# OllieBoyne/sslap

Measured on AMD Instinct MI355X. Metric: Medges/s (bid-phase CSR nnz/s) + solve ms, N=200k d=0.1% sparse LAP, higher is better.
Workload: dtype f64

## Files before the change

sslap_amd/auction_solve.py:

```python
import ctypes as C
import os

import numpy as np

from . import _lib

_ENV_DEVICE = "MISSLAP_DEVICE"
_ENV_TAIL = "MISSLAP_TAIL_THRESHOLD"


def _options(problem, eps_start, max_iter, device=None, tail_threshold=None, profile=None, force_f64=False,
             input_on_device=False, shard=None, rounds_per_sync=None, tiled_min_k=None, tiled_shape=None, shard_min_k=None,
             engine=None, cand=None, nnz_limit=None, cand_build_max_k=None, cand_refresh=None,
             input_stream=None):
    if problem not in ("min", "max"):
        problem = "max" if problem != "min" else "min"
    o = _lib.Options()
    o.struct_size = C.sizeof(_lib.Options)
    o.device = int(os.environ.get(_ENV_DEVICE, 0)) if device is None else int(device)
    o.maximize = 1 if problem == "max" else 0
    o.eps_start = float(np.float32(eps_start))
    o.max_iter = int(max_iter)
    o.input_on_device = 1 if input_on_device else 0
    o.input_stream = None if input_stream is None else C.c_void_p(int(input_stream))
# ... 10 lines not shown
    o.shard_min_K = 0 if shard_min_k is None else int(shard_min_k)
    c = 1 if cand is None else int(cand)
    o.cand_mode = 1 if c == 0 else (2 if c == 2 else 0)
    o.partial_in_list_order = 0
    o.cand_build_max_K = 0 if cand_build_max_k is None else int(cand_build_max_k)
    o.cand_refresh_min = 0 if cand_refresh is None else int(cand_refresh) + 1
    o.nnz_limit = 0 if nnz_limit is None else int(nnz_limit)
    return o


class AuctionSolver:

    def __init__(self, loc, val, num_rows=0, num_cols=0, problem="min", max_iter=1000000, eps_start=0,
                 **gpu_opts):
        lib = _lib.load()
        loc, val = self._check_buffers(loc, val)
        self._h = C.c_void_p()
        self._opts = _options(problem, eps_start, max_iter, **gpu_opts)
        self._problem = problem
        loc_c = np.ascontiguousarray(loc)
        val_c = np.ascontiguousarray(val)
        _lib.check(lib.misslap_create(C.byref(self._h), loc_c.shape[0], loc_c.ctypes.data, val_c.ctypes.data,
                                      C.byref(self._opts)))
        if problem == "min":
            np.multiply(val, -1, out=val)
        self._post_create()

    @classmethod
    def _from_handle(cls, handle, opts, problem):
        self = cls.__new__(cls)
        self._h, self._opts, self._problem = handle, opts, problem
        self._post_create()
        return self

    @classmethod
    def from_dense(cls, mat, problem="min", max_iter=1000000, eps_start=0, **gpu_opts):
        lib = _lib.load()
        h = C.c_void_p()
        opts = _options(problem, eps_start, max_iter, **gpu_opts)
        matc = np.ascontiguousarray(mat)
        nnz = C.c_int64(-1)
        rc = lib.misslap_create_dense(C.byref(h), matc.shape[0], matc.shape[1], matc.ctypes.data, C.byref(opts),
                                      C.byref(nnz))
        return rc, h, opts, int(nnz.value)

    @classmethod
    def from_device_pointers(cls, loc_ptr, val_ptr, nnz, problem="min", max_iter=1000000, eps_start=0,
                             **gpu_opts):
        lib = _lib.load()
        h = C.c_void_p()
        opts = _options(problem, eps_start, max_iter, input_on_device=True, **gpu_opts)
        _lib.check(lib.misslap_create(C.byref(h), int(nnz), C.c_void_p(int(loc_ptr)), C.c_void_p(int(val_ptr)),
                                      C.byref(opts)))
        return cls._from_handle(h, opts, problem)

    @staticmethod
    def _check_buffers(loc, val):
        if not isinstance(loc, np.ndarray) or not isinstance(val, np.ndarray):
            raise TypeError("loc and val must be numpy arrays")
        if loc.ndim != 2:
            raise ValueError(f"Buffer has wrong number of dimensions (expected 2, got {loc.ndim})")
        if loc.dtype != np.int32:
            raise ValueError(f"Buffer dtype mismatch, expected 'DTYPE_int_t' but got '{loc.dtype.name}'")
        if val.ndim != 1:
            raise ValueError(f"Buffer has wrong number of dimensions (expected 1, got {val.ndim})")
        if val.dtype != np.float64:
            raise ValueError(f"Buffer dtype mismatch, expected 'DTYPE_t' but got '{_cname(val.dtype)}'")
        if loc.shape[1] != 2 or loc.shape[0] != val.shape[0]:
            raise ValueError("loc must have shape (nnz, 2) and val shape (nnz,)")
        return loc, val

    def _post_create(self):
        lib = _lib.load()
        n, m, z = C.c_int64(), C.c_int64(), C.c_int64()
        _lib.check(lib.misslap_dims(self._h, C.byref(n), C.byref(m), C.byref(z)))
        self.num_rows, self.num_cols, self.nnz = n.value, m.value, z.value
        st = self.status()
        self.tail_threshold, self.rounds_per_sync = int(st.tail_threshold), int(st.rounds_per_sync)
        self.shard_min_K = int(st.shard_min_K)
        self.meta = {"start_eps": round(float(st.eps), 3)}
        self.gpu = {}

    def __del__(self):
        h = getattr(self, "_h", None)
        if h:
            try:
                _lib.load().misslap_destroy(h)
            except Exception:
                pass
            self._h = None

    def solve(self):
        lib = _lib.load()
        sol = np.empty(self.num_rows, dtype=np.int32)
        meta = _lib.new_meta()
        _lib.check(lib.misslap_solve(self._h, sol.ctypes.data, C.byref(meta)))
        self._fill_meta(meta)
        return sol

    @staticmethod
    def solve_batch(solvers, group_size=0):
        lib = _lib.load()
        n = len(solvers)
        sols = [np.empty(s.num_rows, dtype=np.int32) for s in solvers]
        handles = (C.c_void_p * n)(*[s._h for s in solvers])
        outs = (C.c_void_p * n)(*[a.ctypes.data for a in sols])
        metas = (_lib.Meta * n)()
        for m in metas:
            m.struct_size = C.sizeof(_lib.Meta)
        info = _lib.BatchInfo()
        meta_ptrs = (C.POINTER(_lib.Meta) * n)(*[C.pointer(m) for m in metas])
        _lib.check(lib.misslap_solve_batch(handles, n, outs, meta_ptrs, int(group_size), C.byref(info)))
        for s, m in zip(solvers, metas):
            s._fill_meta(m)
        return sols, dict(groups=int(info.groups), calls_recorded=int(info.calls_recorded),
                          launches_issued=int(info.launches_issued), wall_ms=float(info.wall_ms),
                          host_ms=dict(fibers=round(float(info.host_ms_fibers), 3), flush=round(float(info.host_ms_flush), 3),
                                       wait=round(float(info.host_ms_wait), 3)))

    def solve_sharded(self, comm=None):
        lib = _lib.load()
        sol = np.empty(self.num_rows, dtype=np.int32)
        meta = _lib.new_meta()
        _lib.check(lib.misslap_solve_sharded(self._h, comm._c if comm is not None else None, sol.ctypes.data,
                                             C.byref(meta)))
        self._fill_meta(meta)
        return sol

    def _fill_meta(self, m):
        self.meta["start_eps"] = round(float(m.start_eps), 3)
        self.meta["eCE"] = int(m.eCE)
        self.meta["its"] = int(m.its)
        self.meta["nreductions"] = int(m.nreductions)
        self.meta["soln_found"] = int(m.soln_found)
        self.meta["n_assigned"] = int(m.n_assigned)
        self.meta["obj"] = round(float(m.obj_f32), 3)
        self.meta["final_eps"] = round(float(m.final_eps), 3)
        self.meta["timer"] = {"setup": f"{m.setup_ms:.2f}ms", "solve": f"{m.solve_ms:.2f}ms"}
        g = dict(obj_f64=float(m.obj_f64), edges_scanned=int(m.edges_scanned), bids_made=int(m.bids_made),
                 grid_rounds=int(m.grid_rounds), tail_rounds=int(m.tail_rounds), bytes_per_edge=int(m.bytes_per_edge),
                 setup_ms=float(m.setup_ms), solve_ms=float(m.solve_ms), final_eps_f32=float(m.final_eps),
                 start_eps_f32=float(m.start_eps), tail_edges=int(m.tail_edges), shard_edges=int(m.shard_edges),
                 tiled_active=int(m.tiled_active), tiled_min_K=int(m.tiled_min_K),
                 cand_hits=int(m.cand_hits), cand_edges=int(m.cand_edges), lines_active=int(m.lines_active),
                 sharded_rounds=int(m.sharded_rounds), tiled_format=int(m.tiled_format),
                 phases_with_lines=int(m.phases_with_lines), eps_phases=int(m.eps_phases),
                 filter_undecided=int(m.filter_undecided),
                 complete_assignment=tuple(bool(m.complete_assignment >> k & 1) for k in range(3)),
                 valid_assignment=bool(m.valid_assignment))
        d = [float(x) for x in m.tail_stats]
        g["tail_modes"] = {name: dict(rounds=int(d[k]), ms=round(d[3 + k] * 1e-5, 3),
                                      us_per_round=round(d[3 + k] * 1e-2 / d[k], 3) if d[k] else None)
                           for k, name in enumerate(("solo", "team", "block"))}
        g["tail_cand"] = dict(bids=int(d[6]), hits=int(d[7]), builds=int(d[8]))
        g["tail_cand_edges"] = int(d[9])
        g["tail_raw"] = d[:6]
        if m.profiled:
            g.update(bid_launches=int(m.bid_launches), bid_ms=float(m.bid_ms), bid_edges=int(m.bid_edges),
                     fullscan_launches=int(m.fullscan_launches), fullscan_ms=float(m.fullscan_ms),
                     fullscan_edges=int(m.fullscan_edges), tail_launches=int(m.tail_launches),
                     tail_ms=float(m.tail_ms), tiled_launches=int(m.tiled_launches), tiled_ms=float(m.tiled_ms),
                     tiled_edges=int(m.tiled_edges), bid_edges_read=int(m.bid_edges_read),
                     fullscan_edges_read=int(m.fullscan_edges_read))
        self.gpu = g
        self.meta["gpu"] = g

    @property
    def prices(self):
        p = np.empty(self.num_cols, dtype=np.float64)
        _lib.check(_lib.load().misslap_get_prices(self._h, p.ctypes.data, 0))
        return p

    def update_values(self, val):
        if not isinstance(val, np.ndarray):
            raise TypeError("val must be a numpy array")
        if val.dtype != np.float64:
            raise ValueError(f"Buffer dtype mismatch, expected 'double' but got '{_cname(val.dtype)}'")
        delta = C.c_double(0.0)
        if val.ndim == 2:
            shape = getattr(self, "_dense_shape", None)
            if shape is None:
                raise ValueError("an (N, M) matrix updates a solver made by from_matrix only; pass the nnz values instead")
            if val.shape != shape:
                raise ValueError(f"matrix of shape {val.shape}, the solver was made from one of shape {shape}")
            v = np.ascontiguousarray(val)
            if np.isposinf(v).any():
                raise ValueError("the matrix holds +inf")
            _lib.check(_lib.load().misslap_update_dense(self._h, v.ctypes.data, 0, None, C.byref(delta)))
            return float(delta.value)
        if val.ndim != 1:
            raise ValueError(f"Buffer has wrong number of dimensions (expected 1, got {val.ndim})")
        if val.shape[0] != self.nnz:
            raise ValueError(f"{val.shape[0]} values given, the solver holds {self.nnz} entries")
        v = np.ascontiguousarray(val)
        if not np.isfinite(v).all():
            raise ValueError("val holds a NaN or an infinity")
        _lib.check(_lib.load().misslap_update_values(self._h, v.ctypes.data, self.nnz, 0, None, C.byref(delta)))
        return float(delta.value)

    def update_values_device(self, ptr, input_stream=None, dense=False):
        delta = C.c_double(0.0)
        stream = None if input_stream is None else C.c_void_p(int(input_stream))
        lib = _lib.load()
        if dense:
            _lib.check(lib.misslap_update_dense(self._h, C.c_void_p(int(ptr)), 1, stream, C.byref(delta)))
        else:
            _lib.check(lib.misslap_update_values(self._h, C.c_void_p(int(ptr)), self.nnz, 1, stream, C.byref(delta)))
        return float(delta.value)

    def resolve(self, prices=None, eps_start=0):
        e = float(eps_start)
        if e != e:
            raise ValueError("eps_start is NaN")
        ptr, on_device = None, 0
        if prices is not None:
            if isinstance(prices, np.ndarray):
                if prices.dtype != np.float64:
                    raise ValueError(f"Buffer dtype mismatch, expected 'double' but got '{_cname(prices.dtype)}'")
                p = np.ascontiguousarray(prices)
                bad_nan, bad_sign = not np.isfinite(p).all(), bool(np.signbit(p).any())
                ptr = p.ctypes.data
            elif hasattr(prices, "data_ptr") and getattr(prices, "is_cuda", False):
                import torch
                if prices.dtype != torch.float64:
                    raise ValueError(f"prices must be float64, got {prices.dtype}")
                p = prices.contiguous()
                bad_nan, bad_sign = not bool(torch.isfinite(p).all()), bool(torch.signbit(p).any())
                ptr, on_device = p.data_ptr(), 1
            else:
                raise TypeError("prices must be a numpy array or a tensor on the device")
            if p.ndim != 1 or p.shape[0] != self.num_cols:
                raise ValueError(f"prices must have shape ({self.num_cols},), got {tuple(p.shape)}")
            if bad_nan:
                raise ValueError("prices hold a NaN or an infinity")
            if bad_sign:
                raise ValueError("prices must be >= 0 (with the sign bit clear: -0.0 is rejected)")
        lib = _lib.load()
        sol = np.empty(self.num_rows, dtype=np.int32)
        meta = _lib.new_meta()
        _lib.check(lib.misslap_resolve(self._h, None if ptr is None else C.c_void_p(ptr), on_device, float(np.float32(e)),
                                       sol.ctypes.data, C.byref(meta)))
        self._fill_meta(meta)
        return sol

    def status(self):
        st = _lib.Status()
        _lib.check(_lib.load().misslap_get_status(self._h, C.byref(st)))
        return st

    def state(self):
        st = self.status()
        p = np.empty(self.num_cols, dtype=np.float64)
        U = np.empty(self.num_rows, dtype=np.int32)
        p2o = np.empty(self.num_rows, dtype=np.int32)
        o2p = np.empty(self.num_cols, dtype=np.int32)
        _lib.check(_lib.load().misslap_get_state(self._h, p.ctypes.data, U.ctypes.data, p2o.ctypes.data,
                                                 o2p.ctypes.data))
        return dict(K=int(st.K), U=U[:st.K].copy(), p=p, p2o=p2o, o2p=o2p, eps=float(st.eps), its=int(st.its),
                    nreductions=int(st.nreductions))

    def round_bid(self):
        _lib.check(_lib.load().misslap_round_bid(self._h))

    def round_tiebreak(self):
        _lib.check(_lib.load().misslap_round_tiebreak(self._h))

    def round_apply(self):
        _lib.check(_lib.load().misslap_round_apply(self._h))

    def run_tail(self):
        _lib.check(_lib.load().misslap_run_tail(self._h))

    def phase_end(self):
        fin = C.c_int32(0)
        _lib.check(_lib.load().misslap_phase_end(self._h, C.byref(fin)))
        return bool(fin.value)

    def check_ece(self, eps):
        ok = C.c_int32(0)
        _lib.check(_lib.load().misslap_check_ece(self._h, float(np.float32(eps)), C.byref(ok)))
        return bool(ok.value)

    def finish(self):
        sol = np.empty(self.num_rows, dtype=np.int32)
        meta = _lib.new_meta()
        _lib.check(_lib.load().misslap_finish(self._h, sol.ctypes.data, C.byref(meta)))
        self._fill_meta(meta)
        return sol

    def exchange_buffers(self):
        k, p, n = C.c_void_p(), C.c_void_p(), C.c_int64()
        _lib.check(_lib.load().misslap_exchange_buffers(self._h, C.byref(k), C.byref(p), C.byref(n)))
        return k.value, p.value, n.value

    def matching_cardinality(self):
        size = C.c_int32()
        _lib.check(_lib.load().misslap_matching_of(self._h, C.byref(size), None))
        return int(size.value)

    def set_stream(self, hip_stream):
        _lib.check(_lib.load().misslap_set_stream(self._h, C.c_void_p(int(hip_stream))))


def _cname(dt):
    return {"float32": "float", "float64": "double", "int64": "long", "int32": "int"}.get(dt.name, dt.name)

# ... 91 lines not shown
```

sslap_amd/csrc/kernels_tail.hpp:

```cpp
#pragma once
#include "device_common.hpp"

namespace misslap {

struct TailArgs {
    Ctl *ctl;
    const int *row_ptr;
    double *price;
    PriceRec *rec;
    int *p2o;
    int *o2p;
    int *U;
    int2 *cand;
    double *cand64;
    int thr;
    int round_budget;
    float eps;
};

constexpr int kHashSize = 2048;

__device__ __forceinline__ unsigned long long readlane_u64(unsigned long long v, int l) {
    const int lo = __builtin_amdgcn_readlane((int)(unsigned)(v & 0xffffffffull), l);
    const int hi = __builtin_amdgcn_readlane((int)(unsigned)(v >> 32), l);
// ... 668 lines not shown
    __syncthreads();
#ifdef MISSLAP_TAIL_STAMP_TEAM
    unsigned long long sacc[8] = {0, 0, 0, 0, 0, 0, 0, 0}, sprev = __builtin_amdgcn_s_memtime();
    const CycleStamp stamp{sacc, &sprev, wave == 0};
#else
    const NoStamp stamp;
#endif
    const int rmax = round_limit(nits, max_iter);
    int r = 0;
    int par = 0;
    const int ls = min(lane, kTeamMax - 1);
    PriceRec grec = PriceRec{0.0, -1, 0};
    bool have_g = false;
    for (;;) {
        if (n0 >= K) {
            if (lane == 0) {
                sU[n0] = -1;
                sStart[n0] = 0;
            }
            tail_barrier_lds();
            nits += r;
            return true;
        }
        int sp = -2;
        LaneBid w = {};
        stamp.light(0);
        if (!have_g) grec = cand_gather1(slot, cls, src);
#ifdef MISSLAP_TAIL_STAMP_TEAM
        asm volatile("s_waitcnt vmcnt(0)" ::: "memory");
        stamp.light(1);
#endif
        cand_eval1_lane(slot, grec, cls, eps, w, st.bad_hi, [&](int prev) {
            sp = prev;
            request(sp);
        });
        bool publish = w.mine;
        double bid = w.bid;
        int obj = w.obj, own = grec.owner, ost = grec.ostart, len = w.len;
        int nprev = w.prev, npst = w.pstart;
        if (!w.hit) {
            CandBid b;
            CandBuildArgs bd;
            const typename E::Raw none[4] = {};
            const int e = a.row_ptr[pi + 1 + lane_zero()];
            wave_bid_full<E, RecSource, true, false>(ed, src, ps, e, none, eps, b, bd, st.err);
            st.misses += 1;
            st.miss_edges += (unsigned long long)b.len;
            if (bd.want) tail_build(a, pi, bd, eps, st);
            publish = lane == 0;
            bid = key_to_bid(b.key);
            obj = b.obj;
            own = nprev = b.prev;
            ost = npst = b.pstart;
            len = b.len;
        }
        st.edges += (unsigned long long)len;
        st.bids += 1;
        stamp.light(2);
        if (publish) {
            const int old = atomicExch(&L.tab[pipe_hash(obj)], r);
            PriceRec mine;
            mine.price = bid;
            mine.owner = pi;
            mine.ostart = ps;
            L.slot[par][n0].rec = mine;
            L.slot[par][n0].aux = make_int4(obj, own, ost, 0);
            if (old == r || own < 0) L.dirty[par] = r;
        }
        stamp.light(3);
        tail_barrier_lds();
        stamp.light(4);
        {
            const int dflag = L.dirty[par];
            const PriceRec lrec = L.slot[par][ls].rec;
            const int lobj = L.slot[par][ls].aux.x;
#ifdef MISSLAP_TAIL_STAMP_TEAM
            asm volatile("s_waitcnt lgkmcnt(0)" ::: "memory");
            stamp.light(5);
#endif
            if (__builtin_amdgcn_readfirstlane(dflag) != r) {
                have_g = sp == nprev;
                if (have_g) {
                    touch_slot(slot);
                    if (lane < K) a.rec[lobj] = lrec;
                    grec = cand_gather1(slot, cls, src);
                } else {
                    if (lane < K) a.rec[lobj] = lrec;
                }
                pi = nprev;
                ps = npst;
            } else {
                have_g = false;
                const bool act = lane < K;
                const int4 laux = L.slot[par][ls].aux;
                const unsigned long long lkey = act ? bid_to_key(lrec.price) : 0ull;
                const int lo = act ? laux.x : (-2 - lane);
                const int lprev = act ? laux.y : 0, lpst = act ? laux.z : 0;
                int u = act ? lrec.owner : -1;
                int sx = act ? lrec.ostart : 0;
                bool lose = false;
                for (int m = 0; m < K; ++m) {
                    const int om = __builtin_amdgcn_readlane(lo, m);
                    const bool same = (om == lo) && (m != lane);
                    if (__any(same)) {
                        const unsigned long long km = readlane_u64(lkey, m);
                        lose |= same && (km > lkey || (km == lkey && m < lane));
                    }
                }
                const bool won = act && !lose;
                if (won) apply_winner(a, u, sx, lo, lprev, lkey);
                u = won ? lprev : u;
                sx = won ? lpst : sx;
                const unsigned long long kmask = (1ull << K) - 1ull;
                const unsigned long long holes = __ballot(act && u == -1) & kmask;
                const int Kn = K - __popcll(holes);
                const unsigned long long lmask = (1ull << Kn) - 1ull;
                unsigned long long hl = holes & lmask;
                unsigned long long mv = ~holes & ~lmask & kmask;
                while (hl) {
                    const int hk = __ffsll((long long)hl) - 1, mk = __ffsll((long long)mv) - 1;
                    const int mu = __builtin_amdgcn_readlane(u, mk), ms = __builtin_amdgcn_readlane(sx, mk);
                    if (lane == hk) {
                        u = mu;
                        sx = ms;
                    }
                    hl &= hl - 1;
                    mv &= mv - 1;
                }
                K = Kn;
                pi = n0 < K ? __builtin_amdgcn_readlane(u, min(n0, kWave - 1)) : -1;
                ps = n0 < K ? __builtin_amdgcn_readlane(sx, min(n0, kWave - 1)) : 0;
            }
        }
        par ^= 1;
        r += 1;
        const bool done = K <= 2 || r >= rmax;
        if (!done && n0 < K && sp != pi) request(pi);
        stamp.light(6);
        if (done) break;
    }
    nits += r;
#ifdef MISSLAP_TAIL_STAMP_TEAM
    if (threadIdx.x == 0)
        for (int k = 1; k <= 6; ++k) a.ctl->dbg[5 + k] += sacc[k];
#endif
    if (lane == 0 && n0 < kTeamMax) {
        sU[n0] = pi;
        sStart[n0] = ps;
    }
    __syncthreads();
    return false;
}

template <class E, int kThreads, bool kTeamOnly = false>
struct k_tail {
    MISSLAP_KERNEL(kThreads)
    static __device__ __forceinline__ void run(TailArgs a, E ed) {
        static_assert(!kTeamOnly || (kThreads == 2 * kTailMax && kThreads / kWave == kTeamMax), "one slot per wavefront");
        constexpr bool kBlockOnly = kThreads > kTailMax && !kTeamOnly;
        constexpr bool kDuoOnly = kThreads == kWave;
        static_assert(!kDuoOnly || !kTeamOnly, "roles are exclusive");
        __shared__ int sU[kTailMax];
        __shared__ unsigned long long sKey[kTailMax];
        __shared__ int sObj[kTailMax];
        __shared__ int sPrev[kTailMax];
        __shared__ int sStart[kTailMax];
        __shared__ int sPst[kTailMax];
        __shared__ int sList[kTailMax];
        __shared__ int hObj[kHashSize];
        __shared__ unsigned long long hKey[kHashSize];
        __shared__ int hPos[kHashSize];
        __shared__ int sCnt[3][kThreads / kWave];
        __shared__ int sK, sMissCnt;
        __shared__ long long sNits;

        Ctl *ctl = a.ctl;
        const int t = threadIdx.x, lane = t & 63, wave = t >> 6;
        constexpr int nwaves = kThreads / kWave;
        int K = ctl->K;
        long long nits = ctl->nits;
        const long long max_iter =
            a.round_budget > 0 ? min(ctl->max_iter, nits + (long long)(kBlockOnly ? max(a.round_budget / 4, 1) : a.round_budget))
                               : ctl->max_iter;
        if (K == 0 || K > a.thr || nits >= max_iter) return;
        if (kBlockOnly && K <= kTeamMax) return;
        if (kTeamOnly && (K <= 2 || K > kTeamMax)) return;
        if (kDuoOnly && (K > 2 || !E::kCand || a.cand == nullptr)) return;
        if (!kBlockOnly && !kTeamOnly && a.round_budget > 0 && K > 2 && E::kCand && a.cand != nullptr) return;
        const int K0 = K;
        const long long nits0 = nits;
        for (int n = t; n < kTailMax; n += kThreads) {
            sU[n] = (n < K) ? a.U[n] : -1;
            sStart[n] = (n < K) ? a.row_ptr[sU[n]] : 0;
        }
        if (!kDuoOnly)
            for (int h = t; h < kHashSize; h += kThreads) {
                hObj[h] = -1;
                hKey[h] = 0ull;
                hPos[h] = kPosNone;
            }
        const double eps = (double)a.eps;
        TailStats st;
        st.edges = st.miss_edges = st.builds = 0ull;
        st.bids = st.misses = st.bad_hi = 0u;
        st.err = 0;
        st.hint = 0.0;
        if (t == 0) sMissCnt = 0;
        __syncthreads();

        unsigned long long md[6] = {0, 0, 0, 0, 0, 0};
#ifdef MISSLAP_TAIL_STAMP_BLOCK
        unsigned long long bacc[8] = {0, 0, 0, 0, 0, 0, 0, 0};
#endif
        auto mode_begin = [&](int m) {
            md[3 + m] -= __builtin_amdgcn_s_memrealtime();
            md[m] -= (unsigned long long)nits;
        };
        auto mode_end = [&](int m) {
            md[3 + m] += __builtin_amdgcn_s_memrealtime();
            md[m] += (unsigned long long)nits;
        };
        auto flush_stats = [&]() {
            const bool bad_bid = __any(bad_hi_is_error(st.bad_hi));
            if (lane == 0) {
                if (st.bids) {
                    const unsigned long long hits = (unsigned long long)(st.bids - st.misses), hit_edges = st.edges - st.miss_edges;
                    atomicAdd(&ctl->edges, st.edges);
                    atomicAdd(&ctl->tail_edges, st.edges);
                    atomicAdd(&ctl->bids, (unsigned long long)st.bids);
                    if (hits) {
                        atomicAdd(&ctl->cand_hits, hits);
                        atomicAdd(&ctl->cand_edges, hit_edges);
                    }
                    atomicAdd(&ctl->dbg[12], (unsigned long long)st.bids);
                    atomicAdd(&ctl->dbg[13], hits);
                    atomicAdd(&ctl->dbg[14], st.builds);
                    atomicAdd(&ctl->dbg[15], hit_edges);
                }
                if (bad_bid) st.err |= kErrNegativeBid;
                if (st.err) atomicOr(&ctl->err, st.err);
            }
        };
        for (;;) {
            if (kBlockOnly && K <= kTeamMax) break;
            if (kDuoOnly) {
                mode_begin(0);
                tail_pair_mode(a, ed, sU, sStart, K, nits, max_iter, eps, st);
                mode_end(0);
                break;
            }
            if (kTeamOnly) {
                if (K > 2 && nits < max_iter) {
                    mode_begin(1);
                    if (tail_team1_pipe(a, ed, sU, sStart, K, nits, max_iter, eps, st)) {
                        flush_stats();
                        return;
                    }
                    mode_end(1);
                }
                break;
            }
            if (!kBlockOnly && K <= 2) {
                if (wave == 0) {
                    mode_begin(0);
                    tail_solo_mode(a, ed, sU, sStart, K, nits, max_iter, eps, st);
                    mode_end(0);
                    if (lane == 0) {
                        sK = K;
                        sNits = nits;
                    }
                }
                __syncthreads();
                K = sK;
                nits = sNits;
                break;
            }
            if (!kBlockOnly && K <= kTeamMax) {
                mode_begin(1);
                tail_team_mode(a, ed, sU, sStart, K, nits, max_iter, eps, st);
                mode_end(1);
                if (K == 0 || nits >= max_iter) break;
                continue;
            }
            mode_begin(2);
#ifdef MISSLAP_TAIL_STAMP_BLOCK
            unsigned long long sprev_b = __builtin_amdgcn_s_memtime();
            const CycleStamp bstamp{bacc, &sprev_b, wave == 0};
#else
            const NoStamp bstamp;
#endif
            {
                const RecSource src{a.rec};
                constexpr int kBlockDepth = kBlockOnly ? 1 : 3;
                const int wv = __builtin_amdgcn_readfirstlane(wave);
                for (int base = 0; base < K; base += kBlockDepth * 2 * nwaves) {
                    typename E::Slot sl[kBlockDepth];
                    PriceRec rr[kBlockDepth];
#pragma unroll
                    for (int c = 0; c < kBlockDepth; ++c) {
                        const int nme = base + c * 2 * nwaves + 2 * wv + (lane >> 5);
                        const int pme = nme < K ? sU[min(nme, kTailMax - 1)] : -1;
                        sl[c] = cand_no_line<typename E::Slot>();
                        if (E::kCand && a.cand != nullptr) sl[c] = line_of<E>(a, pme, lane & (kCandLanes - 1));
                    }
                    bstamp(1);
#pragma unroll
                    for (int c = 0; c < kBlockDepth; ++c) {
                        const int n0 = base + c * 2 * nwaves + 2 * wv;
                        if (E::kCand) rr[c] = cand_gather2(sl[c], n0 < K, n0 + 1 < K, src);
                    }
                    bstamp(2);
#pragma unroll
                    for (int c = 0; c < kBlockDepth; ++c) {
                        const int n0 = base + c * 2 * nwaves + 2 * wv;
                        if (n0 >= K) continue;
                        LaneBid2 w;
                        w.hit = false;
                        w.hm = 0ull;
                        w.len[0] = w.len[1] = 0;
                        if (E::kCand) cand_eval2_lane(sl[c], rr[c], true, n0 + 1 < K, eps, w, st.bad_hi);
                        if (w.hit) {
                            const int n = n0 + (lane >> 5);
                            sKey[n] = bid_to_key(w.bid);
                            sObj[n] = sl[c].x;
                            sPrev[n] = rr[c].owner;
                            sPst[n] = rr[c].ostart;
                        }
                        if (__popcll(w.hm) == 2) {
                            st.edges += (unsigned long long)(w.len[0] + w.len[1]);
                            st.bids += 2;
                        } else {
                            const bool h0 = (unsigned)w.hm != 0u, h1 = (unsigned)(w.hm >> 32) != 0u;
                            if (h0) {
                                st.edges += (unsigned long long)w.len[0];
                                st.bids += 1;
                            } else if (lane == 0) {
                                sList[atomicAdd(&sMissCnt, 1)] = n0;
                            }
                            if (n0 + 1 < K) {
                                if (h1) {
                                    st.edges += (unsigned long long)w.len[1];
                                    st.bids += 1;
                                } else if (lane == 0) {
                                    sList[atomicAdd(&sMissCnt, 1)] = n0 + 1;
                                }
                            }
                        }
                    }
#ifdef MISSLAP_TAIL_STAMP_BLOCK
                    bstamp.light(3);
#endif
                }
                __syncthreads();
                bstamp(3);
                const int nmiss = sMissCnt;
                for (int m = wave; m < nmiss; m += nwaves) {
                    const int n = __builtin_amdgcn_readfirstlane(sList[m]);
                    const int i = __builtin_amdgcn_readfirstlane(sU[n]);
                    const int s0 = __builtin_amdgcn_readfirstlane(sStart[n]);
                    const typename E::Raw none[4] = {};
                    const int ev = a.row_ptr[i + 1 + lane_zero()];
                    CandBid bm;
                    CandBuildArgs ba;
                    wave_bid_full<E, RecSource, true, false>(ed, src, s0, ev, none, eps, bm, ba, st.err);
                    ba.want = ba.want && a.cand != nullptr;
                    if (lane == 0) {
                        sKey[n] = bm.key;
                        sObj[n] = bm.obj;
                        sPrev[n] = bm.prev;
                        sPst[n] = bm.pstart;
                    }
                    st.edges += (unsigned long long)bm.len;
                    st.miss_edges += (unsigned long long)bm.len;
                    st.bids += 1;
                    st.misses += 1;
                    if (ba.want) tail_build(a, i, ba, eps, st);
                }
            }
            __syncthreads();
            bstamp(4);

            if (K <= kWave) {
                if (wave == 0) {
                    const bool act = lane < K;
                    const unsigned long long key = act ? sKey[lane] : 0ull;
                    const int obj = act ? sObj[lane] : (-2 - lane);
                    bool lose = false;
                    int hs = 0;
                    bool dup = false;
                    if (act) {
                        hs = (int)(((unsigned)obj * 2654435761u) >> 21) & (kHashSize - 1);
                        for (;;) {
                            const int old = atomicCAS(&hObj[hs], -1, obj);
                            if (old == -1) break;
                            if (old == obj) {
                                dup = true;
                                break;
                            }
                            hs = (hs + 1) & (kHashSize - 1);
                        }
                    }
                    const bool contested = __any(dup);
                    __builtin_amdgcn_fence(__ATOMIC_RELEASE, "wavefront");
                    __builtin_amdgcn_wave_barrier();
                    if (act && !dup) hObj[hs] = -1;
                    if (contested) {
                        for (int m = 0; m < K; ++m) {
                            const int om = __builtin_amdgcn_readlane(obj, m);
                            const bool same = (om == obj) && (m != lane);
                            if (__any(same)) {
                                const unsigned long long km = readlane_u64(key, m);
                                lose |= same && (km > key || (km == key && m < lane));
                            }
                        }
                    }
                    int u = act ? sU[lane] : -1;
                    int sx = act ? sStart[lane] : 0;
                    if (act && !lose) {
                        u = apply_winner(a, u, sx, obj, sPrev[lane], key);
                        sx = sPst[lane];
                    }
                    const unsigned long long kmask = (K >= 64) ? ~0ull : ((1ull << K) - 1ull);
                    const unsigned long long holes = __ballot(act && u == -1) & kmask;
                    const int Kn = K - __popcll(holes);
                    const unsigned long long lmask = (Kn >= 64) ? ~0ull : ((1ull << Kn) - 1ull);
                    const unsigned long long hl = holes & lmask;
                    if (hl == 0ull) {
                        if (act) {
                            sU[lane] = (lane < Kn) ? u : -1;
                            sStart[lane] = sx;
                        }
                    } else {
                        const unsigned long long mv = ~holes & ~lmask & kmask;
                        const bool is_hl = (hl >> lane) & 1ull, is_mv = (mv >> lane) & 1ull;
                        if (is_hl) sList[__popcll(hl & lanemask_lt())] = lane;
                        __builtin_amdgcn_fence(__ATOMIC_RELEASE, "wavefront");
                        __builtin_amdgcn_wave_barrier();
                        __builtin_amdgcn_fence(__ATOMIC_ACQUIRE, "wavefront");
                        if (is_mv) {
                            const int dst = sList[__popcll(mv & lanemask_lt())];
                            sU[dst] = u;
                            sStart[dst] = sx;
                        }
                        if (act) {
                            if (lane >= Kn) sU[lane] = -1;
                            else if (!is_hl) {
                                sU[lane] = u;
                                sStart[lane] = sx;
                            }
                        }
                    }
                    if (lane == 0) {
                        sK = Kn;
                        sMissCnt = 0;
                    }
                }
            } else {
                const bool act = t < K;
                unsigned long long key = 0ull;
                int obj = -1, h = 0;
                if (act) {
                    key = sKey[t];
                    obj = sObj[t];
                    h = (int)(((unsigned)obj * 2654435761u) >> 21) & (kHashSize - 1);
                    for (;;) {
                        const int old = atomicCAS(&hObj[h], -1, obj);
                        if (old == -1 || old == obj) break;
                        h = (h + 1) & (kHashSize - 1);
                    }
                    atomicMax(&hKey[h], key);
                }
                __syncthreads();
                if (act && hKey[h] == key) atomicMin(&hPos[h], t);
                __syncthreads();
                const bool win = act && hPos[h] == t;
                __syncthreads();
                if (act) {
                    hObj[h] = -1;
                    hKey[h] = 0ull;
                    hPos[h] = kPosNone;
                }
                int u = act ? sU[t] : -1;
                int sx = act ? sStart[t] : 0;
                if (win) {
                    u = apply_winner(a, u, sx, obj, sPrev[t], key);
                    sx = sPst[t];
                }
                const bool hole = act && u == -1;
                const unsigned long long bh = __ballot(hole);
                if (lane == 0) sCnt[0][wave] = __popcll(bh);
                __syncthreads();
                int total = 0;
                for (int w2 = 0; w2 < nwaves; ++w2) total += sCnt[0][w2];
                const int Kn = K - total;
                const bool is_hl = hole && t < Kn;
                const bool is_mv = act && !hole && t >= Kn;
                const unsigned long long bl = __ballot(is_hl), bm = __ballot(is_mv);
                if (lane == 0) {
                    sCnt[1][wave] = __popcll(bl);
                    sCnt[2][wave] = __popcll(bm);
                }
                __syncthreads();
                int pl = __popcll(bl & lanemask_lt()), pm = __popcll(bm & lanemask_lt());
                for (int w2 = 0; w2 < wave; ++w2) {
                    pl += sCnt[1][w2];
                    pm += sCnt[2][w2];
                }
                if (is_hl) sList[pl] = t;
                __syncthreads();
                if (is_mv) {
                    sU[sList[pm]] = u;
                    sStart[sList[pm]] = sx;
                }
                if (act) {
                    if (t >= Kn) sU[t] = -1;
                    else if (!is_hl) {
                        sU[t] = u;
                        sStart[t] = sx;
                    }
                }
                if (t == 0) {
                    sK = Kn;
                    sMissCnt = 0;
                }
            }
            bstamp(5);
            __syncthreads();
            bstamp(6);
            K = sK;
            nits += 1;
            mode_end(2);
            if (K == 0 || nits >= max_iter) break;
        }
        if (t == 0)
            for (int k = 0; k < 6; ++k) ctl->dbg[k] += md[k];
#ifdef MISSLAP_TAIL_STAMP_BLOCK
        if (t == 0)
            for (int k = 1; k <= 6; ++k) ctl->dbg[5 + k] += bacc[k];
#endif

        for (int n = t; n < K0; n += kThreads) a.U[n] = sU[n];
        flush_stats();
        if (t == 0) {
            ctl->K = K;
            ctl->nits = nits;
            ctl->tail_rounds += nits - nits0;
        }
    }
};


}
```

sslap_amd/csrc/misslap.hip:

```cpp
#include <hip/hip_runtime.h>
#include <hip/hip_ext.h>

#include <algorithm>
#include <atomic>
#include <chrono>
#include <cmath>
#include <cstdarg>
#include <cstdio>
#include <cstdlib>
#include <cstring>
#include <initializer_list>
#include <mutex>
#include <thread>
#include <string>
#include <utility>
#include <vector>

#include "../../include/misslap.h"
#include "abi_v1.hpp"
#include "device_common.hpp"
#include "kernels_check.hpp"
#ifdef MISSLAP_DIAG
#include "../../include/misslap_diag.h"
#include "kernels_debug.hpp"
// ... 193 lines not shown
    return launch_tiebreak(h);
}
MISSLAP_API int misslap_round_apply(misslap_solver *h) {
    if (!h) return fail(MISSLAP_ERR_INVALID, "null handle");
    HIP_TRY(hipSetDevice(h->device));
    return launch_apply(h);
}
MISSLAP_API int misslap_run_tail(misslap_solver *h) {
    if (!h) return fail(MISSLAP_ERR_INVALID, "null handle");
    HIP_TRY(hipSetDevice(h->device));
    return launch_tail(h);
}

MISSLAP_API int misslap_get_status(misslap_solver *h, misslap_status *st) {
    if (!h || !st) return fail(MISSLAP_ERR_INVALID, "null argument");
    HIP_TRY(hipSetDevice(h->device));
    int rc = read_ctl(h);
    st->error_bits = h->h_ctl->err;
    st->its = h->h_ctl->nits;
    st->K = h->h_ctl->K;
    st->nreductions = h->nreductions;
    st->eps = h->eps;
    st->target_eps = h->target_eps;
    st->finished = h->finished ? 1 : 0;
    st->tail_threshold = h->thr;
    st->rounds_per_sync = h->rounds_per_sync;
    st->shard_min_K = h->shard_min_K;
    return rc;
}

MISSLAP_API int misslap_check_ece(misslap_solver *h, float eps, int32_t *satisfied) {
    if (!h || !satisfied) return fail(MISSLAP_ERR_INVALID, "null argument");
    HIP_TRY(hipSetDevice(h->device));
    int ok = 0;
    int rc = run_ece(h, eps, &ok);
    *satisfied = ok;
    return rc;
}

MISSLAP_API int misslap_phase_end(misslap_solver *h, int32_t *finished) {
    if (!h) return fail(MISSLAP_ERR_INVALID, "null handle");
    HIP_TRY(hipSetDevice(h->device));
    int rc = read_status(h);
    if (rc) return rc;
    const Ctl &c = *h->h_ctl;
    if (c.nits >= h->max_iter) {
        h->finished = true;
    } else if (c.K == 0) {
        int ok = 0;
        if ((rc = run_ece(h, h->target_eps, &ok))) return rc;
        if (ok) {
            h->finished = true;
        } else if (h->eps < h->target_eps) {
            h->finished = true;
        } else {
            h->eps = h->eps * h->theta;
            launch<k_reset_phase>(h, dim3(blocks_for(h->n_rows > h->n_cols ? h->n_rows : h->n_cols, k_reset_phase::kBlock)), h->ctl, h->p2o,
                                  h->o2p, h->rec, h->U, h->n_rows, h->n_cols);
            HIP_TRY(hipGetLastError());
            h->live_valid = false;
            h->nreductions += 1;
            h->K_ub = h->n_rows;
            h->K_exact = true;
            h->h_ctl->K = h->n_rows;
            h->h_ctl->nholes = 0;
            h->h_ctl->nleft = 0;
            h->phase_fresh = true;
            h->ece_flag_clear = true;
            begin_phase(h);
        }
    }
    if (finished) *finished = h->finished ? 1 : 0;
    return MISSLAP_OK;
}

MISSLAP_API int misslap_finish(misslap_solver *h, int32_t *person_to_object_out, misslap_meta *meta_out) {
    if (!h) return fail(MISSLAP_ERR_INVALID, "null handle");
    HIP_TRY(hipSetDevice(h->device));
    int rc;
    if ((rc = read_ctl(h))) return rc;
    const bool complete = h->h_ctl->K == 0;
    h->ctl_fresh = false;
    launch_alone(h, nullptr, k_final_reset, dim3(1), dim3(1), 0, h->ctl);
    const FinalOut fo{1, h->maximize, h->o2p, h->contrib, h->nmatch, h->n_rows, h->n_cols, h->fin_slots};
    int n_slots = 0;
    HIP_TRY(stream_memset(h, h->fin_slots, 0, sizeof(FinSlot) * (size_t)h->fin_slots_n));
    if ((rc = launch_rows_all(h, h->target_eps, fo, &n_slots))) return rc;
    h->ece_flag_clear = false;
    if (h->f32) {
        EdgesF32 ed{h->edges32};
        launch_alone(h, nullptr, k_obj_sum<EdgesF32>, dim3(1), dim3(1024), 0, h->ctl, ed, h->row_ptr, h->p2o, h->n_rows, h->maximize,
                     h->contrib, h->nmatch, h->fin_slots, n_slots);
    } else {
        EdgesF64 ed{h->col, h->val64};
        launch_alone(h, nullptr, k_obj_sum<EdgesF64>, dim3(1), dim3(1024), 0, h->ctl, ed, h->row_ptr, h->p2o, h->n_rows, h->maximize,
                     h->contrib, h->nmatch, h->fin_slots, n_slots);
    }
    HIP_TRY(hipGetLastError());
    if (person_to_object_out)
        HIP_TRY(stream_memcpy(h, person_to_object_out, h->p2o, sizeof(int) * (size_t)h->n_rows, hipMemcpyDeviceToHost));
    launch_alone(h, nullptr, k_collect_stats, dim3(1), dim3(1024), 0, h->ctl, h->wg_stats, h->wg_stats_slots);
    HIP_TRY(hipGetLastError());
    h->ctl_fresh = false;
    if ((rc = read_ctl(h))) return rc;
    const int ece = complete && !h->h_ctl->ece_fail ? 1 : 0;
    if (!meta_out) return MISSLAP_OK;
    size_t out_bytes = sizeof(misslap_meta_v1);
    if (h->abi >= 2) {
        const int32_t sz = meta_out->struct_size;
        if (sz < (int32_t)offsetof(misslap_meta, edges_scanned) || sz > 65536)
            return fail(MISSLAP_ERR_INVALID, "misslap_meta.struct_size = %d: set it to sizeof(misslap_meta) before the call", sz);
        out_bytes = std::min<size_t>((size_t)sz, sizeof(misslap_meta));
    }
    const Ctl &c = *h->h_ctl;
    misslap_meta full;
    misslap_meta *meta = &full;
    std::memset(meta, 0, sizeof(*meta));
    meta->struct_size = (int32_t)out_bytes;
    meta->abi_version = MISSLAP_ABI_VERSION;
    {
        const unsigned long long distinct = c.val_cnt[0], n_neg = c.val_cnt[1], n_big = c.val_cnt[2], n_invalid = c.val_cnt[3];
        const unsigned long long uniq = distinct + (n_neg ? 1ull : 0ull);
        meta->complete_assignment = (uniq == (unsigned long long)h->n_rows ? 1 : 0) | (n_neg == 0 ? 2 : 0) | (n_big == 0 ? 4 : 0);
        meta->valid_assignment = n_invalid == 0 ? 1 : 0;
        meta->lines_active = (h->cand != nullptr && !h->lines_dropped) ? 1 : 0;
    }
    meta->start_eps = h->start_eps;
    meta->final_eps = h->eps;
    meta->target_eps = h->target_eps;
    meta->eCE = ece;
    meta->soln_found = (c.K == 0) ? ece : 0;
    meta->nreductions = h->nreductions;
    meta->its = c.nits;
    meta->n_assigned = (int64_t)h->n_rows - c.K;
    meta->n_rows = h->n_rows;
    meta->n_cols = h->n_cols;
    meta->nnz = h->nnz;
    meta->obj_f64 = c.obj;
    meta->obj_f32 = (float)c.obj;
    meta->setup_ms = h->setup_ms;
    meta->solve_ms = h->solve_ms;
    meta->edges_scanned = c.edges;
    meta->bids_made = c.bids;
    meta->grid_rounds = c.grid_rounds;
    meta->tail_rounds = c.tail_rounds;
    meta->tail_edges = c.tail_edges;
    meta->bytes_per_edge = h->f32 ? 8 : 12;
    meta->profiled = h->profile ? 1 : 0;
    meta->tiled_active = h->tiled_ok ? 1 : 0;
    meta->tiled_min_K = h->tiled_min_K;
    meta->shard_edges = c.shard_edges;
    for (int k = 0; k < 6; ++k) meta->tail_stats[k] = (double)c.dbg[k];
    for (int k = 0; k < 4; ++k) meta->tail_stats[6 + k] = (double)c.dbg[12 + k];
#if defined(MISSLAP_TAIL_STAMP) || defined(MISSLAP_TAIL_STAMP_SOLO) || defined(MISSLAP_TAIL_STAMP_TEAM) || \
    defined(MISSLAP_TAIL_STAMP_BLOCK) || defined(MISSLAP_TILED_STAMP) || defined(MISSLAP_TAIL_STAMP_DUO)
    for (int k = 0; k < 6; ++k) meta->tail_stats[k] = (double)c.dbg[6 + k];
#endif
    meta->cand_hits = c.cand_hits;
    meta->cand_edges = c.cand_edges;
    meta->sharded_rounds = h->sharded_rounds;
    meta->tiled_format = h->tiled_ok ? h->tiled_fmt : 0;
    meta->phases_with_lines = h->phases_with_lines;
    meta->eps_phases = h->phases_run;
    meta->filter_undecided = -1;
    if (h->profile && h->prof_used) {
        std::vector<unsigned long long> le(2 * (size_t)h->launch_idx);
        if (h->launch_idx)
            HIP_TRY(hipMemcpy(le.data(), h->launch_edges, sizeof(unsigned long long) * le.size(),
                              hipMemcpyDeviceToHost));
        for (size_t k = 0; k < h->prof_used; ++k) {
            const ProfRec &r = h->prof[k];
            float ms = 0.f;
            if (hipEventElapsedTime(&ms, r.start, r.stop) != hipSuccess) continue;
            if (r.kind == 0 || r.kind == 2) {
                const unsigned long long e = le[2 * (size_t)r.launch_idx], eh = le[2 * (size_t)r.launch_idx + 1];
                if (r.kind == 0) {
                    meta->bid_launches += 1;
                    meta->bid_ms += ms;
                    meta->bid_edges += e;
                    meta->bid_edges_read += e - eh;
                } else {
                    meta->tiled_launches += 1;
                    meta->tiled_ms += ms;
                    meta->tiled_edges += e;
                }
                if (r.fullscan) {
                    meta->fullscan_launches += 1;
                    meta->fullscan_ms += ms;
                    meta->fullscan_edges += e;
                    meta->fullscan_edges_read += e - (r.kind == 0 ? eh : 0ull);
                }
            } else {
                meta->tail_launches += 1;
                meta->tail_ms += ms;
            }
        }
    }
    if (h->abi >= 2) {
        std::memcpy(meta_out, &full, out_bytes);
    } else {
        misslap_meta_v1 v1;
        static_assert(offsetof(misslap_meta, complete_assignment) - offsetof(misslap_meta, start_eps) == sizeof(misslap_meta_v1),
                      "misslap_meta = {struct_size, abi_version} + the version-1 fields + appended fields");
        std::memcpy(&v1, &full.start_eps, sizeof(v1));
        v1.merge_launches = 0;
        v1.merge_ms = 0.0;
        std::memcpy(meta_out, &v1, sizeof(v1));
    }
    return MISSLAP_OK;
}

misslap_round_ops handle_round_ops(misslap_solver *h) {
    misslap_round_ops o;
    std::memset(&o, 0, sizeof(o));
    o.struct_size = (int32_t)sizeof(o);
    o.tail_threshold = h->thr;
    o.shard_min_K = h->shard_min_K;
    o.rounds_per_sync = h->rounds_per_sync_auto && !h->live_off ? kRoundsPerSyncLive : h->rounds_per_sync;
    o.large_round_K = kRoundSmallMax;
    o.rounds_per_sync_large = kRoundsPerSyncLargeK;
    o.max_iter = h->max_iter;
    o.ctx = h;
    o.status = [](void *x, int64_t *K, int64_t *its) {
        misslap_solver *s = static_cast<misslap_solver *>(x);
        const int rc = read_status(s);
        *K = s->h_ctl->K;
        *its = s->h_ctl->nits;
        return rc;
    };
    o.status_post = [](void *x, int32_t slot) { return status_enqueue(static_cast<misslap_solver *>(x), slot & 1); };
    o.status_take = [](void *x, int32_t slot, int64_t *K, int64_t *its) {
        misslap_solver *s = static_cast<misslap_solver *>(x);
        const int rc = status_wait(s, slot & 1);
        *K = s->h_stat[slot & 1].K;
        *its = s->h_stat[slot & 1].nits;
        return rc;
    };
    o.round_bid = [](void *x) { return launch_bid(static_cast<misslap_solver *>(x)); };
    o.round_tiebreak = [](void *x) { return launch_tiebreak(static_cast<misslap_solver *>(x)); };
    o.round_apply = [](void *x) { return launch_apply(static_cast<misslap_solver *>(x)); };
    o.run_tail = [](void *x) { return launch_tail(static_cast<misslap_solver *>(x)); };
    o.phase_end = [](void *x, int32_t *fin) { return misslap_phase_end(static_cast<misslap_solver *>(x), fin); };
    o.best_key = h->best_key;
    o.best_pos = h->best_pos;
    o.n_objects = h->n_cols;
    o.stream = h->stream;
    return o;
}

MISSLAP_API int misslap_solve(misslap_solver *h, int32_t *person_to_object_out, misslap_meta *meta) {
    if (!h) return fail(MISSLAP_ERR_INVALID, "null handle");
    if (h->world != 1) return fail(MISSLAP_ERR_STATE, "misslap_solve drives one GPU; sharded handles use misslap_solve_sharded");
    return misslap_solve_sharded(h, nullptr, person_to_object_out, meta);
}
#include "abi_comm.hpp"
#include "abi_batch.hpp"

MISSLAP_API int misslap_get_state(misslap_solver *h, double *prices, int32_t *unassigned, int32_t *person_to_object,
                                  int32_t *object_to_person) {
    if (!h) return fail(MISSLAP_ERR_INVALID, "null handle");
    HIP_TRY(hipSetDevice(h->device));
    HIP_TRY(hipStreamSynchronize(h->stream));
    if (prices) HIP_TRY(hipMemcpy(prices, h->price, sizeof(double) * (size_t)h->n_cols, hipMemcpyDeviceToHost));
    if (unassigned) HIP_TRY(hipMemcpy(unassigned, h->U, sizeof(int) * (size_t)h->n_rows, hipMemcpyDeviceToHost));
    if (person_to_object)
        HIP_TRY(hipMemcpy(person_to_object, h->p2o, sizeof(int) * (size_t)h->n_rows, hipMemcpyDeviceToHost));
    if (object_to_person)
        HIP_TRY(hipMemcpy(object_to_person, h->o2p, sizeof(int) * (size_t)h->n_cols, hipMemcpyDeviceToHost));
    return MISSLAP_OK;
}
#include "abi_diag.hpp"
#include "abi_warm.hpp"
#include "abi_batch_common.hpp"
#include "abi_batch_stream.hpp"
#include "abi_dense_batch.hpp"
#include "abi_dense_batch_status.hpp"
#include "abi_sparse_batch.hpp"
#include "abi_matching_batch.hpp"
#include "abi_ell_batch.hpp"
#include "abi_sparse_batch_status.hpp"
```

Before: 5385.

## Add clean-round fast path and early candidate line prefetch to block tail

In the block-mode tail auction, each round now tags hits and inserts bid objects into a tagged LDS hash using atomicMax to detect conflicting bids on the same object or bids on unowned objects. When a round has no conflicts, winners are applied directly and the hash-based conflict resolution, compaction and extra barriers are skipped. Candidate lines for the first sweep are also prefetched from the previous round's displaced owners, reusing them when the bidder matches. This adds per-round LDS atomics and register state, a hash clear on the dirty path, and a new clean-round counter statistic.

After: 5460 (median of 6 runs). 1.4% higher.

```diff
diff --git a/sslap_amd/auction_solve.py b/sslap_amd/auction_solve.py
--- a/sslap_amd/auction_solve.py
+++ b/sslap_amd/auction_solve.py
@@ -186,6 +186,7 @@
         g["tail_modes"] = {name: dict(rounds=int(d[k]), ms=round(d[3 + k] * 1e-5, 3),
                                       us_per_round=round(d[3 + k] * 1e-2 / d[k], 3) if d[k] else None)
                            for k, name in enumerate(("solo", "team", "block"))}
+        g["tail_modes"]["block"]["clean_rounds"] = int(d[10])
         g["tail_cand"] = dict(bids=int(d[6]), hits=int(d[7]), builds=int(d[8]))
         g["tail_cand_edges"] = int(d[9])
         g["tail_raw"] = d[:6]
diff --git a/sslap_amd/csrc/kernels_tail.hpp b/sslap_amd/csrc/kernels_tail.hpp
--- a/sslap_amd/csrc/kernels_tail.hpp
+++ b/sslap_amd/csrc/kernels_tail.hpp
@@ -844,6 +844,29 @@
     return false;
 }
 
+constexpr int kCleanTab = kHashSize;
+constexpr int kCleanProbes = 8;
+static_assert(2 * kCleanTab == kPipeTab, "clean_hash: pipe_hash's top 11 bits");
+__device__ __forceinline__ int clean_hash(int obj) { return pipe_hash(obj) >> 1; }
+__device__ __forceinline__ int slot_index_here(int t) {
+    asm volatile("" : "+v"(t));
+    return t;
+}
+__device__ __forceinline__ void lds_landed_here(int &a, int &b) { asm volatile("" : "+v"(a), "+v"(b)); }
+__device__ __forceinline__ bool clean_insert(unsigned long long *tab, unsigned tag, int obj) {
+    const unsigned long long first = (unsigned long long)tag << 32;
+    unsigned long long cur = first | (unsigned long long)(unsigned)obj;
+    int h = clean_hash(obj);
+    for (int probe = 0; probe < kCleanProbes; ++probe) {
+        const unsigned long long old = atomicMax(&tab[h], cur);
+        if (old < first) return false;
+        if (old == cur || (unsigned)(old >> 32) != tag) return true;
+        cur = min(old, cur);
+        h = (h + 1) & (kCleanTab - 1);
+    }
+    return true;
+}
+
 template <class E, int kThreads, bool kTeamOnly = false>
 struct k_tail {
     MISSLAP_KERNEL(kThreads)
@@ -863,6 +886,9 @@
         __shared__ unsigned long long hKey[kHashSize];
         __shared__ int hPos[kHashSize];
         __shared__ int sCnt[3][kThreads / kWave];
+        unsigned long long *const cTab = hKey;
+        __shared__ unsigned sHit[kTailMax];
+        __shared__ unsigned sDirty;
         __shared__ int sK, sMissCnt;
         __shared__ long long sNits;
 
@@ -885,12 +911,15 @@
             sU[n] = (n < K) ? a.U[n] : -1;
             sStart[n] = (n < K) ? a.row_ptr[sU[n]] : 0;
         }
+        if (!kDuoOnly && !kTeamOnly)
+            for (int n = t; n < kTailMax; n += kThreads) sHit[n] = 0u;
         if (!kDuoOnly)
             for (int h = t; h < kHashSize; h += kThreads) {
                 hObj[h] = -1;
                 hKey[h] = 0ull;
                 hPos[h] = kPosNone;
             }
+        if (!kDuoOnly && !kTeamOnly && t == 0) sDirty = 0u;
         const double eps = (double)a.eps;
         TailStats st;
         st.edges = st.miss_edges = st.builds = 0ull;
@@ -933,6 +962,23 @@
                 if (st.err) atomicOr(&ctl->err, st.err);
             }
         };
+#ifndef MISSLAP_TAIL_BLOCK_EARLY_SWEEPS
+#define MISSLAP_TAIL_BLOCK_EARLY_SWEEPS 1
+#endif
+        constexpr int kEarlySweeps = (kBlockOnly && E::kCand) ? MISSLAP_TAIL_BLOCK_EARLY_SWEEPS : 0;
+        constexpr bool kEarly = kEarlySweeps > 0;
+        constexpr int kEarlyN = kEarly ? kEarlySweeps : 1;
+        unsigned rtag = 0u;
+        unsigned long long nclean = 0ull;
+        typename E::Slot el[kEarlyN];
+        int enp[kEarlyN];
+        if (!kDuoOnly && !kTeamOnly) {
+#pragma unroll
+            for (int q = 0; q < kEarlyN; ++q) {
+                el[q] = cand_no_line<typename E::Slot>();
+                enp[q] = -2;
+            }
+        }
         for (;;) {
             if (kBlockOnly && K <= kTeamMax) break;
             if (kDuoOnly) {
@@ -975,6 +1021,7 @@
                 continue;
             }
             mode_begin(2);
+            rtag += 1u;
 #ifdef MISSLAP_TAIL_STAMP_BLOCK
             unsigned long long sprev_b = __builtin_amdgcn_s_memtime();
             const CycleStamp bstamp{bacc, &sprev_b, wave == 0};
@@ -993,7 +1040,20 @@
                         const int nme = base + c * 2 * nwaves + 2 * wv + (lane >> 5);
                         const int pme = nme < K ? sU[min(nme, kTailMax - 1)] : -1;
                         sl[c] = cand_no_line<typename E::Slot>();
-                        if (E::kCand && a.cand != nullptr) sl[c] = line_of<E>(a, pme, lane & (kCandLanes - 1));
+                        if (E::kCand && a.cand != nullptr) {
+                            if (kEarly && c == 0 && base < kEarlySweeps * 2 * nwaves) {
+                                int ep = -2;
+#pragma unroll
+                                for (int q = 0; q < kEarlyN; ++q)
+                                    if (base == q * 2 * nwaves) {
+                                        sl[c] = el[q];
+                                        ep = enp[q];
+                                    }
+                                if (pme != ep) sl[c] = line_of<E>(a, pme, lane & (kCandLanes - 1));
+                            } else {
+                                sl[c] = line_of<E>(a, pme, lane & (kCandLanes - 1));
+                            }
+                        }
                     }
                     bstamp(1);
 #pragma unroll
@@ -1011,12 +1071,28 @@
                         w.hm = 0ull;
                         w.len[0] = w.len[1] = 0;
                         if (E::kCand) cand_eval2_lane(sl[c], rr[c], true, n0 + 1 < K, eps, w, st.bad_hi);
+                        if (kEarly && c == 0 && base < kEarlySweeps * 2 * nwaves) {
+                            int o = -2;
+                            const bool both = a.cand != nullptr && __popcll(w.hm) == 2;
+                            if (both) {
+                                const int o0 = __builtin_amdgcn_readlane(rr[c].owner, __ffs((int)(unsigned)w.hm) - 1);
+                                const int o1 = __builtin_amdgcn_readlane(rr[c].owner, __ffs((int)(unsigned)(w.hm >> 32)) + (kCandLanes - 1));
+                                o = lane < kCandLanes ? o0 : o1;
+                            }
+#pragma unroll
+                            for (int q = 0; q < kEarlyN; ++q)
+                                if (base == q * 2 * nwaves) {
+                                    if (both) el[q] = line_of<E>(a, o, lane & (kCandLanes - 1));
+                                    enp[q] = o >= 0 ? o : -2;
+                                }
+                        }
                         if (w.hit) {
                             const int n = n0 + (lane >> 5);
                             sKey[n] = bid_to_key(w.bid);
                             sObj[n] = sl[c].x;
                             sPrev[n] = rr[c].owner;
                             sPst[n] = rr[c].ostart;
+                            sHit[n] = rtag;
                         }
                         if (__popcll(w.hm) == 2) {
                             st.edges += (unsigned long long)(w.len[0] + w.len[1]);
@@ -1043,8 +1119,16 @@
                     bstamp.light(3);
 #endif
                 }
-                __syncthreads();
+                if (kEarly) tail_barrier_lds();
+                else __syncthreads();
                 bstamp(3);
+                if (t < K) {
+                    const int ts = slot_index_here(t);
+                    const unsigned hit_t = sHit[ts];
+                    int obj_t = sObj[ts], prev_t = sPrev[ts];
+                    lds_landed_here(obj_t, prev_t);
+                    if (hit_t == rtag && (clean_insert(cTab, rtag, obj_t) || prev_t < 0)) sDirty = rtag;
+                }
                 const int nmiss = sMissCnt;
                 for (int m = wave; m < nmiss; m += nwaves) {
                     const int n = __builtin_amdgcn_readfirstlane(sList[m]);
@@ -1067,16 +1151,36 @@
                     st.bids += 1;
                     st.misses += 1;
                     if (ba.want) tail_build(a, i, ba, eps, st);
-                }
-            }
-            __syncthreads();
+                    if (lane == 0 && (clean_insert(cTab, rtag, bm.obj) || bm.prev < 0)) sDirty = rtag;
+                }
+            }
+            if (kEarly) tail_barrier_lds();
+            else __syncthreads();
             bstamp(4);
 
-            if (K <= kWave) {
+            const int dirty = (int)sDirty;
+            const int tf = slot_index_here(min(t, kTailMax - 1));
+            int fu = -1, fs = 0, fo = 0, fp = 0, fq = 0;
+            unsigned long long fk = 0ull;
+            if (t < K) {
+                fu = sU[tf], fs = sStart[tf], fo = sObj[tf], fp = sPrev[tf], fq = sPst[tf];
+                fk = sKey[tf];
+                lds_landed_here(fu, fs);
+            }
+            const bool clean = (unsigned)__builtin_amdgcn_readfirstlane(dirty) != rtag;
+            if (clean) {
+                if (t < K) {
+                    sU[tf] = apply_winner(a, fu, fs, fo, fp, fk);
+                    sStart[tf] = fq;
+                }
+                if (t == 0) sMissCnt = 0;
+                nclean += 1ull;
+            } else if (K <= kWave) {
                 if (wave == 0) {
                     const bool act = lane < K;
-                    const unsigned long long key = act ? sKey[lane] : 0ull;
-                    const int obj = act ? sObj[lane] : (-2 - lane);
+                    const int ln = slot_index_here(lane);
+                    const unsigned long long key = act ? sKey[ln] : 0ull;
+                    const int obj = act ? sObj[ln] : (-2 - lane);
                     bool lose = false;
                     int hs = 0;
                     bool dup = false;
@@ -1106,11 +1210,11 @@
                             }
                         }
                     }
-                    int u = act ? sU[lane] : -1;
-                    int sx = act ? sStart[lane] : 0;
+                    int u = act ? sU[ln] : -1;
+                    int sx = act ? sStart[ln] : 0;
                     if (act && !lose) {
-                        u = apply_winner(a, u, sx, obj, sPrev[lane], key);
-                        sx = sPst[lane];
+                        u = apply_winner(a, u, sx, obj, sPrev[ln], key);
+                        sx = sPst[ln];
                     }
                     const unsigned long long kmask = (K >= 64) ? ~0ull : ((1ull << K) - 1ull);
                     const unsigned long long holes = __ballot(act && u == -1) & kmask;
@@ -1119,8 +1223,8 @@
                     const unsigned long long hl = holes & lmask;
                     if (hl == 0ull) {
                         if (act) {
-                            sU[lane] = (lane < Kn) ? u : -1;
-                            sStart[lane] = sx;
+                            sU[ln] = (lane < Kn) ? u : -1;
+                            sStart[ln] = sx;
                         }
                     } else {
                         const unsigned long long mv = ~holes & ~lmask & kmask;
@@ -1135,10 +1239,10 @@
                             sStart[dst] = sx;
                         }
                         if (act) {
-                            if (lane >= Kn) sU[lane] = -1;
+                            if (lane >= Kn) sU[ln] = -1;
                             else if (!is_hl) {
-                                sU[lane] = u;
-                                sStart[lane] = sx;
+                                sU[ln] = u;
+                                sStart[ln] = sx;
                             }
                         }
                     }
@@ -1148,12 +1252,15 @@
                     }
                 }
             } else {
+                for (int h = t; h < kHashSize; h += kThreads) hKey[h] = 0ull;
+                __syncthreads();
                 const bool act = t < K;
+                const int tn = slot_index_here(t);
                 unsigned long long key = 0ull;
                 int obj = -1, h = 0;
                 if (act) {
-                    key = sKey[t];
-                    obj = sObj[t];
+                    key = sKey[tn];
+                    obj = sObj[tn];
                     h = (int)(((unsigned)obj * 2654435761u) >> 21) & (kHashSize - 1);
                     for (;;) {
                         const int old = atomicCAS(&hObj[h], -1, obj);
@@ -1172,11 +1279,11 @@
                     hKey[h] = 0ull;
                     hPos[h] = kPosNone;
                 }
-                int u = act ? sU[t] : -1;
-                int sx = act ? sStart[t] : 0;
+                int u = act ? sU[tn] : -1;
+                int sx = act ? sStart[tn] : 0;
                 if (win) {
-                    u = apply_winner(a, u, sx, obj, sPrev[t], key);
-                    sx = sPst[t];
+                    u = apply_winner(a, u, sx, obj, sPrev[tn], key);
+                    sx = sPst[tn];
                 }
                 const bool hole = act && u == -1;
                 const unsigned long long bh = __ballot(hole);
@@ -1205,10 +1312,10 @@
                     sStart[sList[pm]] = sx;
                 }
                 if (act) {
-                    if (t >= Kn) sU[t] = -1;
+                    if (t >= Kn) sU[tn] = -1;
                     else if (!is_hl) {
-                        sU[t] = u;
-                        sStart[t] = sx;
+                        sU[tn] = u;
+                        sStart[tn] = sx;
                     }
                 }
                 if (t == 0) {
@@ -1219,7 +1326,7 @@
             bstamp(5);
             __syncthreads();
             bstamp(6);
-            K = sK;
+            if (!clean) K = sK;
             nits += 1;
             mode_end(2);
             if (K == 0 || nits >= max_iter) break;
@@ -1229,6 +1336,10 @@
 #ifdef MISSLAP_TAIL_STAMP_BLOCK
         if (t == 0)
             for (int k = 1; k <= 6; ++k) ctl->dbg[5 + k] += bacc[k];
+#endif
+#if !defined(MISSLAP_TAIL_STAMP) && !defined(MISSLAP_TAIL_STAMP_SOLO) && !defined(MISSLAP_TAIL_STAMP_DUO) && \
+    !defined(MISSLAP_TAIL_STAMP_TEAM) && !defined(MISSLAP_TAIL_STAMP_BLOCK) && !defined(MISSLAP_TILED_STAMP)
+        if (!kDuoOnly && !kTeamOnly && t == 0) ctl->dbg[6] += nclean;
 #endif
 
         for (int n = t; n < K0; n += kThreads) a.U[n] = sU[n];
diff --git a/sslap_amd/csrc/misslap.hip b/sslap_amd/csrc/misslap.hip
--- a/sslap_amd/csrc/misslap.hip
+++ b/sslap_amd/csrc/misslap.hip
@@ -369,9 +369,11 @@
     meta->shard_edges = c.shard_edges;
     for (int k = 0; k < 6; ++k) meta->tail_stats[k] = (double)c.dbg[k];
     for (int k = 0; k < 4; ++k) meta->tail_stats[6 + k] = (double)c.dbg[12 + k];
+    meta->tail_stats[10] = (double)c.dbg[6];
 #if defined(MISSLAP_TAIL_STAMP) || defined(MISSLAP_TAIL_STAMP_SOLO) || defined(MISSLAP_TAIL_STAMP_TEAM) || \
     defined(MISSLAP_TAIL_STAMP_BLOCK) || defined(MISSLAP_TILED_STAMP) || defined(MISSLAP_TAIL_STAMP_DUO)
     for (int k = 0; k < 6; ++k) meta->tail_stats[k] = (double)c.dbg[6 + k];
+    meta->tail_stats[10] = 0.0;
 #endif
     meta->cand_hits = c.cand_hits;
     meta->cand_edges = c.cand_edges;
```
